# MrinalJain17/CT-image-segmentation

Hardware: AMD Instinct MI355X
Metric: CT volumes/sec training (512x512x48, bs=2/GPU) (higher is better)
Workload: dtype bf16; 1 GPU; 3D U-Net (MONAI UNet, channels 32-64-128-256, 2 res units) training step on 2x1x512x512x48 synthetic CT volumes per GPU (BASELINE.json configs[2]), CrossEntropy + Dice metric + Adam; global_batch=2, parallelism=dp1

## Files before the change

ct-image-segmentation_amd/csrc/conv_halo_sw.hip:

```cpp
#include "conv_common.h"

#ifndef SW_STORE8
#define SW_STORE8 0
#endif
#ifndef SW_FULL_WAIT
#define SW_FULL_WAIT 0
#endif
#ifndef SW_ABL
#define SW_ABL 0
#endif

namespace ctseg {

constexpr int SW_NTHR = 512, SW_TAPB = 8192;

template <int VB, bool UP> struct SwCfg {
  static constexpr bool DENSE = UP && VB == 256;
  static constexpr int TA = (VB == 128 || DENSE) ? 4 : 2;
  static constexpr int O = DENSE ? 1 : 0;
  static constexpr int LB = 10 - O;
  static constexpr int HV = DENSE ? 456 : (TA + 2) * 100;
  static constexpr int NPL = VB / 16, PLANE = HV * 16, HALO = NPL * PLANE;
  static constexpr int CG = VB / 2, CN = SW_TAPB / VB;
  static constexpr int NT = CN / 16;
  static constexpr int RT = TA / 2;
  static constexpr int KS = CG / 32;
  static constexpr int G = DENSE ? 2 : 3;
  static constexpr int NSTAGE = (27 + G - 1) / G;
  static constexpr int WRING = 2 * G * SW_TAPB;
  static constexpr int TOTAL = HALO + WRING + 8 * 3 * CN * 4 + 128 * 4 + 2 * CN * 4;
  static_assert(TOTAL <= 160 * 1024, "LDS");
  __host__ __device__ static constexpr int slot(int ha, int hb, int hc) { return ((ha - O) * LB + (hb - O)) * 10 + hc; }
};

struct SwGeom : TileAxes {};

template <typename H, int VB, bool UP, bool STATS, bool BST = false>
__global__ __launch_bounds__(SW_NTHR) void conv_halo_sw_kernel(const ConvKArgs P, const SwGeom G, int total_tiles) {
  static_assert(!BST || (!STATS && ((UP && VB == 256) || (!UP && VB == 128))), "backward statistics: the input-gradient passes this kernel takes");
  using CF = SwCfg<VB, UP>;
  constexpr int TA = CF::TA, NPL = CF::NPL, PLANE = CF::PLANE, CN = CF::CN, NT = CF::NT, RT = CF::RT, KS = CF::KS;
  constexpr int SW_G = CF::G, SW_NSTAGE = CF::NSTAGE;
  constexpr int O = UP ? 1 : 0;
  constexpr int FA = TA + 2 - O, FB = 10 - O, FV = FA * FB * FB;
  constexpr int NCH = FV * NPL, J = (NCH + SW_NTHR - 1) / SW_NTHR;

  __shared__ __attribute__((aligned(16))) char smem[CF::TOTAL];
  char* const sH = smem;
  char* const sW = smem + CF::HALO;
  float* const sStats = reinterpret_cast<float*>(sW + CF::WRING);
  int* const sTab = reinterpret_cast<int*>(sStats + 8 * 3 * CN);
  float* const sBt = reinterpret_cast<float*>(sTab + 128);

  const int tid = threadIdx.x, lane = tid & 63, wave = tid >> 6;
  const int r16 = lane & 15, q4 = lane >> 4;

  if (tid < 32) {
    int d = 0, wo = 0, kp = 0, cl = 0;
    if (tid < 27) {
      int c = 0, first = 0;
      while (tid >= first + P.cls[c].ntaps) { first += P.cls[c].ntaps; ++c; }
      const int ti = tid - first;
      const int tp = P.cls[c].taps[ti];
      int dv[3] = {tap_dx(tp), tap_dy(tp), tap_dz(tp)};
      d = ((dv[G.pa] * CF::LB + dv[G.pb]) * 10 + dv[G.pc]) * 16;
      wo = (int)(P.cls[c].w_off + (int64_t)ti * CF::CG);
      kp = P.cls[c].kpad;
      cl = c | ((ti == P.cls[c].ntaps - 1) ? 256 : 0);
    }
    sTab[tid] = d; sTab[32 + tid] = wo; sTab[64 + tid] = kp; sTab[96 + tid] = cl;
  }

  constexpr bool LEAN = BST;
  static_assert(!LEAN || (SW_NTHR / 8) % NPL == 0, "lean staging: the plane of a slot must not depend on j");
  int g_byte[LEAN ? 1 : J], g_habc[J], g_lds[LEAN ? 1 : J];
  const int pl0 = (tid >> 3) % NPL;
#pragma unroll
  for (int j = 0; j < J; ++j) {
    const int idx = tid + j * SW_NTHR;
    const int pl = (idx >> 3) % NPL, fv = (idx / (8 * NPL)) * 8 + (idx & 7);
    const int fa = fv / (FB * FB), rem = fv - fa * (FB * FB), fb = rem / FB, fc = rem - fb * FB;
    const int ha = fa + O, hb = fb + O, hc = fc + O;
    g_habc[j] = (fv < FV) ? (ha | (hb << 8) | (hc << 16)) : 0x7f7f7f;
    if constexpr (!LEAN) {
      g_byte[j] = (((ha - 1) * G.ia + (hb - 1) * G.ib + (hc - 1) * G.ic) * P.g_ld + pl * 8) * 2;
      g_lds[j] = pl * PLANE + CF::slot(ha, hb, hc) * 16;
    }
  }
  auto lean_habc = [&](int j, int& ha, int& hb, int& hc) {
    int h = g_habc[j];
    asm volatile("" : "+v"(h));
    ha = h & 0xff; hb = (h >> 8) & 0xff; hc = h >> 16;
  };
  const int64_t in_sample = (int64_t)P.Xi * P.Yi * P.Zi, out_sample = (int64_t)P.Xo * P.Yo * P.Zo;
  u32x4 rh[J];
  auto gload = [&](int t) {
    const auto [n, a0, b0, c0] = tile_origin_abc<TA>(t, G);
    const char* base = P.in + (n * in_sample + (int64_t)a0 * G.ia + (int64_t)b0 * G.ib + (int64_t)c0 * G.ic) * P.g_ld * 2;
#pragma unroll
    for (int j = 0; j < J; ++j) {
      const int ai = a0 - 1 + (g_habc[j] & 0xff), bi = b0 - 1 + ((g_habc[j] >> 8) & 0xff), ci = c0 - 1 + (g_habc[j] >> 16);
      u32x4 v = {0u, 0u, 0u, 0u};
      int gb;
      if constexpr (LEAN) {
        int ha, hb, hc;
        lean_habc(j, ha, hb, hc);
        gb = (((ha - 1) * G.ia + (hb - 1) * G.ib + (hc - 1) * G.ic) * P.g_ld + pl0 * 8) * 2;
      } else {
        gb = g_byte[j];
      }
      if (!(SW_ABL & 16) && (unsigned)ai < (unsigned)G.da && (unsigned)bi < (unsigned)G.db && (unsigned)ci < (unsigned)G.dc)
        v = *reinterpret_cast<const u32x4*>(base + gb);
      rh[j] = v;
    }
  };
  auto sstore = [&]() {
#pragma unroll
    for (int j = 0; j < J; ++j) {
      int gl;
      if constexpr (LEAN) {
        int ha, hb, hc;
        lean_habc(j, ha, hb, hc);
        gl = pl0 * PLANE + CF::slot(ha, hb, hc) * 16;
      } else {
        gl = g_lds[j];
      }
      if ((g_habc[j] & 0xff) != 0x7f) *reinterpret_cast<u32x4*>(sH + gl) = rh[j];
    }
  };

  typedef const __attribute__((address_space(1))) void* gptr_t;
  typedef __attribute__((address_space(3))) void* lptr_t;
  const int w_s64 = tid / (CN * 8), w_row = (tid >> 3) % CN, w_q8 = (tid & 7) ^ ((w_row >> 1) & 7);
  const int w_koff = w_s64 * 64 + w_q8 * 8;
  int wstage = 0;
  auto wload = [&](int stage_in_tile, int slot) {
    char* dst = sW + slot * (SW_G * SW_TAPB) + wave * 1024;
#pragma unroll
    for (int g = 0; g < SW_G; ++g) {
      const int tap = stage_in_tile * SW_G + g;
      if (SW_G * SW_NSTAGE > 27 && tap >= 27) continue;
      if (SW_ABL & 4) continue;
      const char* src = P.w + ((int64_t)sTab[32 + tap] + (int64_t)w_row * sTab[64 + tap] + w_koff) * 2;
      __builtin_amdgcn_global_load_lds((gptr_t)src, (lptr_t)(dst + g * SW_TAPB), 16, 0, 0);
    }
  };

  int pdb, pc;
  patch_voxel(r16, pdb, pc);
  int abase[RT], va[RT], vb[RT];
#pragma unroll
  for (int rt = 0; rt < RT; ++rt) {
    const int wa = (TA == 4) ? (wave >> 1) : (wave >> 2);
    const int i = (TA == 4) ? (2 * (wave & 1) + rt) : (wave & 3);
    va[rt] = wa;
    vb[rt] = 2 * i + pdb;
    abase[rt] = CF::slot(wa + 1, vb[rt] + 1, pc + 1) * 16 + q4 * PLANE;
  }
  const int wrd = r16 * 128, wswz = (r16 >> 1) & 7;
  const bool af32 = P.add_f32 != 0;
  const int ASZ = af32 ? 4 : 2;
  float bias[NT][4];
#pragma unroll
  for (int j = 0; j < NT; ++j)
#pragma unroll
    for (int e = 0; e < 4; ++e) bias[j][e] = (!BST && P.bias != nullptr) ? P.bias[j * 16 + 4 * q4 + e] : 0.f;

  float wsum[NT][4], wsq[NT][4];
#pragma unroll
  for (int j = 0; j < NT; ++j)
#pragma unroll
    for (int e = 0; e < 4; ++e) { wsum[j][e] = 0.f; wsq[j][e] = 0.f; }
  int stat_n = -1;
  auto flush_stats = [&](int n) {
#pragma unroll
    for (int j = 0; j < NT; ++j)
#pragma unroll
      for (int e = 0; e < 4; ++e) {
        float a = wsum[j][e], b = wsq[j][e];
        sum16(a, b);
        if (r16 == 0) {
          const int c = j * 16 + 4 * q4 + e;
          sStats[(wave * 2 + 0) * CN + c] = a;
          sStats[(wave * 2 + 1) * CN + c] = b;
        }
        wsum[j][e] = 0.f;
        wsq[j][e] = 0.f;
      }
    __syncthreads();
    if (tid < 2 * CN) {
      const int which = tid / CN, c = tid % CN;
      float a = 0.f;
#pragma unroll
      for (int w = 0; w < 8; ++w) a += sStats[(w * 2 + which) * CN + c];
      P.stats[stats_slot(P, n, blockIdx.x, which) + c] = a;
    }
    __syncthreads();
  };

  f32x4 acc[RT][NT];
  auto zero_acc = [&]() {
#pragma unroll
    for (int rt = 0; rt < RT; ++rt)
#pragma unroll
      for (int j = 0; j < NT; ++j) acc[rt][j] = f32x4{0.f, 0.f, 0.f, 0.f};
  };
  const int out_sample_bytes = (int)(out_sample * P.o_ld * 2), add_sample_bytes = (int)(out_sample * P.add_ld * ASZ);
  const bool apf = UP && !STATS && P.add != nullptr && !af32;
  int ooff[RT], aoff[RT];
#pragma unroll
  for (int rt = 0; rt < RT; ++rt) {
    const int vox = va[rt] * G.oa + vb[rt] * G.ob + pc * G.oc;
    ooff[rt] = (vox * P.o_ld + 4 * q4) * 2;
    aoff[rt] = (vox * P.add_ld + 4 * q4) * ASZ;
  }
  u32x2 apre[RT][NT];
  constexpr int NQ = NT / 2;
  f32x2 q1[NQ][4], q2[NQ][4];
  float q3 = 0.f;
#pragma unroll
  for (int jp = 0; jp < NQ; ++jp)
#pragma unroll
    for (int h = 0; h < 4; ++h) { q1[jp][h] = f32x2{0.f, 0.f}; q2[jp][h] = f32x2{0.f, 0.f}; }
  const float q_al = BST ? P.bst.alpha[0] : 1.f;
  const int ychunk = (q4 & 1) * 2 + (q4 >> 1);
  const int y_sample_bytes = BST ? (int)(out_sample * P.bst.y_ld * 2) : 0;
  int yoffc[RT];
#pragma unroll
  for (int rt = 0; rt < RT; ++rt) yoffc[rt] = BST ? ((va[rt] * G.oa + vb[rt] * G.ob + pc * G.oc) * P.bst.y_ld + ychunk * 8) * 2 : 0;
  u32x4 ypre[RT];
  int bst_n = -1;
  auto bst_consts = [&](int n) {
    if (tid < 2 * CN) {
      const int c = tid % CN, which = tid / CN;
      const float mean = P.bst.mr[((int64_t)n * P.bst.C + c) * 2], rstd = P.bst.mr[((int64_t)n * P.bst.C + c) * 2 + 1];
      sBt[which * CN + c] = which == 0 ? rstd : -mean * rstd;
    }
    __syncthreads();
  };
  auto bst_chunk = [&](int jp, const u32x4& gz, const u32x4& yv) {
    if (SW_ABL & 128) { q3 += __uint_as_float(gz[0] ^ yv[3]); return; }
    const float* const cb = sBt + jp * 32 + ychunk * 8;
    const f32x4 rs0 = *reinterpret_cast<const f32x4*>(cb), rs1 = *reinterpret_cast<const f32x4*>(cb + 4);
    const f32x4 nm0 = *reinterpret_cast<const f32x4*>(cb + CN), nm1 = *reinterpret_cast<const f32x4*>(cb + CN + 4);
    bst_pair_bf16(gz[0], yv[0], f32x2{rs0[0], rs0[1]}, f32x2{nm0[0], nm0[1]}, q_al, q1[jp][0], q2[jp][0], q3);
    bst_pair_bf16(gz[1], yv[1], f32x2{rs0[2], rs0[3]}, f32x2{nm0[2], nm0[3]}, q_al, q1[jp][1], q2[jp][1], q3);
    bst_pair_bf16(gz[2], yv[2], f32x2{rs1[0], rs1[1]}, f32x2{nm1[0], nm1[1]}, q_al, q1[jp][2], q2[jp][2], q3);
    bst_pair_bf16(gz[3], yv[3], f32x2{rs1[2], rs1[3]}, f32x2{nm1[2], nm1[3]}, q_al, q1[jp][3], q2[jp][3], q3);
  };
  auto flush_bst = [&](int n) {
#pragma unroll
    for (int jp = 0; jp < NQ; ++jp)
#pragma unroll
      for (int h = 0; h < 4; ++h)
#pragma unroll
        for (int e = 0; e < 2; ++e) {
          float a = q1[jp][h][e], b = q2[jp][h][e];
          sum16(a, b);
          if (r16 == 0) {
            sStats[(wave * 3 + 0) * CN + jp * 32 + ychunk * 8 + 2 * h + e] = a;
            sStats[(wave * 3 + 1) * CN + jp * 32 + ychunk * 8 + 2 * h + e] = b;
          }
          q1[jp][h][e] = 0.f; q2[jp][h][e] = 0.f;
        }
    {
      float c = q3;
      sum16(c);
      if (r16 == 0) sStats[(wave * 3 + 2) * CN + ychunk * 8] = c;
      q3 = 0.f;
    }
    __syncthreads();
    if (tid < 3 * CN) {
      const int which = tid / CN, c = tid % CN;
      float a = 0.f;
      if (which < 2 || ((c & 7) == 0 && c < 32)) {
#pragma unroll
        for (int w = 0; w < 8; ++w) a += sStats[(w * 3 + which) * CN + c];
      }
      P.bst.part[bst_slot(P.bst, n, blockIdx.x, which) + c] = a;
    }
    __syncthreads();
  };
  int pend = 0;
  auto class_base = [&](int cls, int a0, int b0, int c0) -> int {
    const ctseg_conv_class& K = P.cls[cls];
    return a0 * G.oa + b0 * G.ob + c0 * G.oc + (K.ox * P.Yo + K.oy) * P.Zo + K.oz;
  };
  auto add_issue = [&](int cls, int n, int a0, int b0, int c0) {
    const int cb = cls >= 0 ? class_base(cls, a0, b0, c0) : 0;
    if (apf) {
      const __amdgpu_buffer_rsrc_t ars = buffer_rsrc(P.add + (int64_t)n * add_sample_bytes, add_sample_bytes);
      const int soff = cb * P.add_ld * ASZ;
#pragma unroll
      for (int rt = 0; rt < RT; ++rt) {
        const bool rv = cls >= 0 && (a0 + va[rt] < G.da) && (b0 + vb[rt] < G.db) && (c0 + pc < G.dc);
#pragma unroll
        for (int j = 0; j < NT; ++j)
          apre[rt][j] = (SW_ABL & 32) ? u32x2{0u, 0u} : __builtin_amdgcn_raw_buffer_load_b64(ars, rv ? aoff[rt] + j * 16 * ASZ : (int)0x80000000, soff, 0);
      }
      pend += RT * NT;
    }
    if constexpr (BST) {
      const __amdgpu_buffer_rsrc_t yrs = buffer_rsrc(P.bst.y + (int64_t)n * y_sample_bytes, y_sample_bytes);
      const int soff = cb * P.bst.y_ld * 2;
#pragma unroll
      for (int rt = 0; rt < RT; ++rt) {
        const bool rv = cls >= 0 && (a0 + va[rt] < G.da) && (b0 + vb[rt] < G.db) && (c0 + pc < G.dc);
        ypre[rt] = (SW_ABL & 64) ? u32x4{1u, 2u, 3u, (uint32_t)soff} : __builtin_amdgcn_raw_buffer_load_b128(yrs, rv ? yoffc[rt] : (int)0x80000000, soff, 0);
      }
      pend += RT;
    }
  };
  auto epilogue = [&](int cls, int next_cls, int n, int a0, int b0, int c0) {
    const int cb = class_base(cls, a0, b0, c0);
    const __amdgpu_buffer_rsrc_t ors = buffer_rsrc(P.out + (int64_t)n * out_sample_bytes, out_sample_bytes);
    const int soff = cb * P.o_ld * 2;
    const int cbq = ((q4 & 1) * 2 + (q4 >> 1)) * 16;
#pragma unroll
    for (int rt = 0; rt < RT; ++rt) {
      const bool rv = (a0 + va[rt] < G.da) && (b0 + vb[rt] < G.db) && (c0 + pc < G.dc);
      u32x2 o2[NT];
#pragma unroll
      for (int j = 0; j < NT; ++j) {
        float v[4];
#pragma unroll
        for (int e = 0; e < 4; ++e) {
          v[e] = acc[rt][j][e] + bias[j][e];
          if (STATS && rv) { wsum[j][e] += v[e]; wsq[j][e] += v[e] * v[e]; }
        }
        if (apf) {
          const u32x2 w2 = apre[rt][j];
          v[0] += h2f<H>(w2[0] & 0xffffu); v[1] += h2f<H>(w2[0] >> 16); v[2] += h2f<H>(w2[1] & 0xffffu); v[3] += h2f<H>(w2[1] >> 16);
        } else if (P.add != nullptr && rv) {
          const char* ap = P.add + (int64_t)n * add_sample_bytes + (int64_t)cb * P.add_ld * ASZ + aoff[rt] + j * 16 * ASZ;
          if (af32) { const f32x4 a4 = *reinterpret_cast<const f32x4*>(ap); v[0] += a4[0]; v[1] += a4[1]; v[2] += a4[2]; v[3] += a4[3]; }
          else {
            const u32x2 w2 = *reinterpret_cast<const u32x2*>(ap);
            v[0] += h2f<H>(w2[0] & 0xffffu); v[1] += h2f<H>(w2[0] >> 16); v[2] += h2f<H>(w2[1] & 0xffffu); v[3] += h2f<H>(w2[1] >> 16);
          }
        }
        o2[j] = u32x2{pack2<H>(v[0], v[1]), pack2<H>(v[2], v[3])};
      }
#if SW_STORE8
#pragma unroll
      for (int j = 0; j < NT; ++j)
        __builtin_amdgcn_raw_buffer_store_b64(o2[j], ors, rv ? ooff[rt] + j * 32 : (int)0x80000000, soff, 0);
      continue;
#endif
#pragma unroll
      for (int jp = 0; jp < NT / 2; ++jp) {
        const auto s0 = __builtin_amdgcn_permlane16_swap(o2[2 * jp][0], o2[2 * jp + 1][0], false, false);
        const auto s1 = __builtin_amdgcn_permlane16_swap(o2[2 * jp][1], o2[2 * jp + 1][1], false, false);
        const u32x4 o4 = {s0[0], s1[0], s0[1], s1[1]};
        const bool keep = rv && (!(SW_ABL & 8) || o4[0] == 0x12345u);
        __builtin_amdgcn_raw_buffer_store_b128(o4, ors, keep ? ooff[rt] - 4 * q4 * 2 + jp * 64 + cbq : (int)0x80000000, soff, 0);
        asm volatile("s_nop 1" ::"v"(o4));
        if constexpr (BST) bst_chunk(jp, rv ? o4 : u32x4{0u, 0u, 0u, 0u}, ypre[rt]);
      }
    }
    pend += RT * NT / 2;
    if (apf || BST) add_issue(next_cls, n, a0, b0, c0);
  };
  auto stage_barrier = [&]() {
    constexpr int YL = BST ? RT : 0, E1 = RT * NT / 2 + YL, E2 = RT * NT / 2 + RT * NT + YL;
    constexpr int T1 = YL, T2 = RT * NT + YL;
    if (SW_FULL_WAIT || pend == 0) asm volatile("s_waitcnt vmcnt(0) lgkmcnt(0)" ::: "memory");
    else if (BST && pend == T1) asm volatile("s_waitcnt vmcnt(%0) lgkmcnt(0)" ::"n"(T1) : "memory");
    else if (BST && pend == T2) asm volatile("s_waitcnt vmcnt(%0) lgkmcnt(0)" ::"n"(T2) : "memory");
    else if (BST && pend == T1 + E1) asm volatile("s_waitcnt vmcnt(%0) lgkmcnt(0)" ::"n"(T1 + E1) : "memory");
    else if (BST && pend == T2 + E2) asm volatile("s_waitcnt vmcnt(%0) lgkmcnt(0)" ::"n"(T2 + E2) : "memory");
    else if (pend == E1) asm volatile("s_waitcnt vmcnt(%0) lgkmcnt(0)" ::"n"(E1) : "memory");
    else if (pend == 2 * E1) asm volatile("s_waitcnt vmcnt(%0) lgkmcnt(0)" ::"n"(2 * E1) : "memory");
    else if (pend == E2) asm volatile("s_waitcnt vmcnt(%0) lgkmcnt(0)" ::"n"(E2) : "memory");
    else if (pend == 2 * E2) asm volatile("s_waitcnt vmcnt(%0) lgkmcnt(0)" ::"n"(2 * E2) : "memory");
    else asm volatile("s_waitcnt vmcnt(0) lgkmcnt(0)" ::: "memory");
    __builtin_amdgcn_s_barrier();
    asm volatile("" ::: "memory");
    pend = 0;
  };

  auto epilogue_plain = [&](int cls, int n, int a0, int b0, int c0) {
    const ctseg_conv_class& K = P.cls[cls];
    int ov[3] = {K.ox, K.oy, K.oz};
    const int64_t obase = n * out_sample + (int64_t)a0 * G.oa + (int64_t)b0 * G.ob + (int64_t)c0 * G.oc +
                          ((int64_t)ov[0] * P.Yo + ov[1]) * P.Zo + ov[2];
#pragma unroll
    for (int rt = 0; rt < RT; ++rt) {
      const bool rv = (a0 + va[rt] < G.da) && (b0 + vb[rt] < G.db) && (c0 + pc < G.dc);
      const int64_t vox = obase + (int64_t)va[rt] * G.oa + (int64_t)vb[rt] * G.ob + (int64_t)pc * G.oc;
#pragma unroll
      for (int j = 0; j < NT; ++j) {
        const int ch = j * 16 + 4 * q4;
        float v[4];
#pragma unroll
        for (int e = 0; e < 4; ++e) {
          v[e] = acc[rt][j][e] + bias[j][e];
          if (STATS && rv) { wsum[j][e] += v[e]; wsq[j][e] += v[e] * v[e]; }
        }
        if (rv) {
          if (P.add != nullptr) {
            const char* ap = P.add + (vox * P.add_ld + ch) * ASZ;
            if (af32) { const f32x4 a4 = *reinterpret_cast<const f32x4*>(ap); v[0] += a4[0]; v[1] += a4[1]; v[2] += a4[2]; v[3] += a4[3]; }
            else {
              const u32x2 w2 = *reinterpret_cast<const u32x2*>(ap);
              v[0] += h2f<H>(w2[0] & 0xffffu); v[1] += h2f<H>(w2[0] >> 16); v[2] += h2f<H>(w2[1] & 0xffffu); v[3] += h2f<H>(w2[1] >> 16);
            }
          }
          *reinterpret_cast<u32x2*>(P.out + (vox * P.o_ld + ch) * 2) = u32x2{pack2<H>(v[0], v[1]), pack2<H>(v[2], v[3])};
        }
      }
    }
  };

  auto epilogue_plain_bst = [&](int n, int a0, int b0, int c0) {
    const ctseg_conv_class& K = P.cls[0];
    const int cb = a0 * G.oa + b0 * G.ob + c0 * G.oc + (K.ox * P.Yo + K.oy) * P.Zo + K.oz;
    const __amdgpu_buffer_rsrc_t ors = buffer_rsrc(P.out + (int64_t)n * out_sample_bytes, out_sample_bytes);
    const __amdgpu_buffer_rsrc_t yrs = buffer_rsrc(P.bst.y + (int64_t)n * y_sample_bytes, y_sample_bytes);
    u32x4 yq[RT][NQ];
#pragma unroll
    for (int rt = 0; rt < RT; ++rt) {
      const bool rv = (a0 + va[rt] < G.da) && (b0 + vb[rt] < G.db) && (c0 + pc < G.dc);
#pragma unroll
      for (int jp = 0; jp < NQ; ++jp) yq[rt][jp] = __builtin_amdgcn_raw_buffer_load_b128(yrs, rv ? yoffc[rt] + jp * 64 : (int)0x80000000, cb * P.bst.y_ld * 2, 0);
    }
    const int cbq = ychunk * 16;
#pragma unroll
    for (int rt = 0; rt < RT; ++rt) {
      const bool rv = (a0 + va[rt] < G.da) && (b0 + vb[rt] < G.db) && (c0 + pc < G.dc);
      u32x2 o2[NT];
#pragma unroll
      for (int j = 0; j < NT; ++j) {
        float v[4];
#pragma unroll
        for (int e = 0; e < 4; ++e) v[e] = acc[rt][j][e];
        if (P.add != nullptr && rv) {
          const char* ap = P.add + (int64_t)n * add_sample_bytes + (int64_t)cb * P.add_ld * ASZ + aoff[rt] + j * 16 * ASZ;
          if (af32) { const f32x4 a4 = *reinterpret_cast<const f32x4*>(ap); v[0] += a4[0]; v[1] += a4[1]; v[2] += a4[2]; v[3] += a4[3]; }
          else {
            const u32x2 w2 = *reinterpret_cast<const u32x2*>(ap);
            v[0] += h2f<H>(w2[0] & 0xffffu); v[1] += h2f<H>(w2[0] >> 16); v[2] += h2f<H>(w2[1] & 0xffffu); v[3] += h2f<H>(w2[1] >> 16);
          }
        }
        o2[j] = u32x2{pack2<H>(v[0], v[1]), pack2<H>(v[2], v[3])};
      }
#pragma unroll
      for (int jp = 0; jp < NQ; ++jp) {
        const auto s0 = __builtin_amdgcn_permlane16_swap(o2[2 * jp][0], o2[2 * jp + 1][0], false, false);
        const auto s1 = __builtin_amdgcn_permlane16_swap(o2[2 * jp][1], o2[2 * jp + 1][1], false, false);
        const u32x4 o4 = {s0[0], s1[0], s0[1], s1[1]};
        __builtin_amdgcn_raw_buffer_store_b128(o4, ors, rv ? ooff[rt] - 4 * q4 * 2 + jp * 64 + cbq : (int)0x80000000, cb * P.o_ld * 2, 0);
        asm volatile("s_nop 1" ::"v"(o4));
        bst_chunk(jp, rv ? o4 : u32x4{0u, 0u, 0u, 0u}, yq[rt][jp]);
      }
    }
  };

  const auto [first, stride, last] = xcd_tile_seq([] { return blockIdx.x; }, gridDim.x, total_tiles);

  __syncthreads();
  int t = first;
  if (t < last) {
    gload(t);
    wload(0, 0);
    sstore();
  }
  __syncthreads();
  for (; t < last; t += stride) {
    const int tn = t + stride;
    const auto [n, a0, b0, c0] = tile_origin_abc<TA>(t, G);
    if (STATS && n != stat_n) {
      if (stat_n >= 0) flush_stats(stat_n);
      stat_n = n;
    }
    if constexpr (BST) {
      if (n != bst_n) {
        if (bst_n >= 0) flush_bst(bst_n);
        bst_n = n;
        bst_consts(n);
      }
    }
    zero_acc();
#pragma unroll 1
    for (int s = 0; s < SW_NSTAGE; ++s) {
      const int slot = wstage & 1;
      if (s + 1 < SW_NSTAGE) wload(s + 1, slot ^ 1);
      else if (tn < last) wload(0, slot ^ 1);
      if (s == 0 && tn < last) gload(tn);
      if ((apf || BST) && s == 0) add_issue(sTab[96] & 255, n, a0, b0, c0);
      const char* wb = sW + slot * (SW_G * SW_TAPB) + wrd;
#pragma unroll
      for (int g = 0; g < SW_G; ++g) {
        const int tap = s * SW_G + g;
        if (SW_G * SW_NSTAGE > 27 && tap >= 27) continue;
        const int delta = sTab[tap];
#pragma unroll
        for (int ks = 0; ks < KS; ++ks) {
          u32x4 xf[RT], wf[NT];
#pragma unroll
          for (int rt = 0; rt < RT; ++rt)
            xf[rt] = (SW_ABL & 2) ? u32x4{(uint32_t)(delta + rt), 1u, 2u, (uint32_t)ks} : *reinterpret_cast<const u32x4*>(sH + abase[rt] + ks * 4 * PLANE + delta);
          const char* wk = wb + g * SW_TAPB + (ks >> 1) * (CN * 128) + (((4 * (ks & 1) + q4) ^ wswz) << 4);
#pragma unroll
          for (int j = 0; j < NT; ++j) wf[j] = (SW_ABL & 2) ? u32x4{(uint32_t)(j + g), 3u, (uint32_t)tap, 5u} : *reinterpret_cast<const u32x4*>(wk + j * 16 * 128);
#pragma unroll
          for (int rt = 0; rt < RT; ++rt)
#pragma unroll
            for (int j = 0; j < NT; ++j) {
              if constexpr ((SW_ABL & 1) != 0) acc[rt][j][0] += __builtin_bit_cast(f32x4, wf[j])[0] * __builtin_bit_cast(f32x4, xf[rt])[1];
              else mma16<H>(acc[rt][j], wf[j], xf[rt]);
            }
        }
        if constexpr (UP) {
          const int cl = sTab[96 + tap];
          if (cl & 256) {
            epilogue(cl & 255, tap + 1 < 27 ? (sTab[96 + tap + 1] & 255) : -1, n, a0, b0, c0);
            zero_acc();
          }
        }
      }
      ++wstage;
      if constexpr (UP) stage_barrier();
      else __syncthreads();
    }
    if constexpr (!UP && BST) epilogue_plain_bst(n, a0, b0, c0);
    else if constexpr (!UP) epilogue_plain(0, n, a0, b0, c0);
    if (tn < last) {
      sstore();
      __syncthreads();
    }
  }
  if (STATS && stat_n >= 0) flush_stats(stat_n);
  if constexpr (BST) { if (bst_n >= 0) flush_bst(bst_n); }
}

static void sw_geom(const ConvKArgs& a, int vb, SwGeom& g) {
  tile_axes_fill(g, a, (vb == 128 || a.sout == 2) ? 4 : 2, 2);
}

bool conv_halo_sw_eligible(const ConvKArgs& a, int dtype, int nclass) {
  if (!is16(dtype) || a.out_f32 || a.sin != 1) return false;
  const int vb = a.Cg * 2;
  if (!((vb == 128 && a.Cn == 64) || (vb == 256 && a.Cn == 32)) || a.Cn_store != a.Cn) return false;
  if ((a.g_ld % 8) != 0 || ((uintptr_t)a.in % 16) != 0 || ((uintptr_t)a.w % 16) != 0) return false;
  if (a.Xr != a.Xi || a.Yr != a.Yi || a.Zr != a.Zi) return false;
  if (sample_bytes(a.Xi, a.Yi, a.Zi, a.g_ld, 2) >= (1ll << 31)) return false;
  if ((int64_t)a.Xr * a.Yr * a.Zr < 2048) return false;
  const bool up = nclass == 8;
  if (up) {
    if (a.sout != 2 || a.Xo != 2 * a.Xr || a.Yo != 2 * a.Yr || a.Zo != 2 * a.Zr) return false;
  } else {
    if (nclass != 1 || a.sout != 1 || a.Xo != a.Xr || a.Yo != a.Yr || a.Zo != a.Zr) return false;
  }
  int taps = 0;
  for (int c = 0; c < nclass; ++c) {
    const ctseg_conv_class& k = a.cls[c];
    if (up ? (k.ntaps != (1 << __builtin_popcount(c))) : (k.ntaps != 27)) return false;
    if (k.kpad < k.ntaps * a.Cg || (k.kpad % 8) != 0 || (k.w_off % 8) != 0) return false;
    if (k.w_off + (int64_t)a.Cn * k.kpad >= (1ll << 31)) return false;
    taps += k.ntaps;
    if (!taps_within(k.taps, k.ntaps, up ? 0 : -1, 1)) return false;
  }
  return taps == 27;
}

static int sw_grid(const ConvKArgs& a, const SwGeom& g) {
  return persistent_grid(CTSEG_NUM_CU, g.tiles * a.N);
}

int conv_halo_sw_slots(const ConvKArgs& a) {
  SwGeom g;
  sw_geom(a, a.Cg * 2, g);
  return sw_grid(a, g);
}

int conv_halo_sw_bst_slots(const ConvKArgs& a, int nclass) {
  if (a.dtype != CTSEG_BF16 || a.stats != nullptr || a.bias != nullptr) return 0;
  if (!((nclass == 8 && a.Cg == 128) || (nclass == 1 && a.Cg == 64))) return 0;
  if (a.bst.C != a.Cn || a.bst.col0 != 0 || a.Cn_store != a.Cn || (a.o_ld % 8) != 0 || ((uintptr_t)a.out % 16) != 0) return 0;
  if ((a.bst.y_ld % 8) != 0 || ((uintptr_t)a.bst.y % 16) != 0) return 0;
  if (sample_bytes(a.Xo, a.Yo, a.Zo, a.bst.y_ld, 2) >= (1ll << 31) || sample_bytes(a.Xo, a.Yo, a.Zo, a.o_ld, 2) >= (1ll << 31)) return 0;
  return conv_halo_sw_slots(a);
}

void launch_conv_halo_sw(ConvKArgs& a, int nclass, hipStream_t st) {
  SwGeom g;
  const int vb = a.Cg * 2;
  sw_geom(a, vb, g);
  a.tiles = g.tiles;
  const int total = g.tiles * a.N;
  const dim3 grid((unsigned)sw_grid(a, g)), blk(SW_NTHR);
  const bool up = nclass == 8, stats = a.stats != nullptr;
  if (a.bst.part != nullptr) {
    if (up) hipLaunchKernelGGL((conv_halo_sw_kernel<BF16, 256, true, false, true>), grid, blk, 0, st, a, g, total);
    else hipLaunchKernelGGL((conv_halo_sw_kernel<BF16, 128, false, false, true>), grid, blk, 0, st, a, g, total);
    return;
  }
  with_storage(a.dtype, [&](auto h, auto vb128, auto up_, auto stats_) {
    constexpr int VB = decltype(vb128)::value ? 128 : 256;
    hipLaunchKernelGGL((conv_halo_sw_kernel<decltype(h), VB, decltype(up_)::value, decltype(stats_)::value>), grid, blk, 0, st, a, g, total);
  }, vb == 128, up, stats);
}

}
```

Measured before the change: 231.7 volumes/s.

## Use triple-buffered weight ring with counted vmcnt waits for plain VB128 conv

```diff
diff --git a/ct-image-segmentation_amd/csrc/conv_halo_sw.hip b/ct-image-segmentation_amd/csrc/conv_halo_sw.hip
--- a/ct-image-segmentation_amd/csrc/conv_halo_sw.hip
+++ b/ct-image-segmentation_amd/csrc/conv_halo_sw.hip
@@ -27,7 +27,8 @@
   static constexpr int KS = CG / 32;
   static constexpr int G = DENSE ? 2 : 3;
   static constexpr int NSTAGE = (27 + G - 1) / G;
-  static constexpr int WRING = 2 * G * SW_TAPB;
+  static constexpr int NSLOT = (!UP && VB == 128) ? 3 : 2;
+  static constexpr int WRING = NSLOT * G * SW_TAPB;
   static constexpr int TOTAL = HALO + WRING + 8 * 3 * CN * 4 + 128 * 4 + 2 * CN * 4;
   static_assert(TOTAL <= 160 * 1024, "LDS");
   __host__ __device__ static constexpr int slot(int ha, int hb, int hc) { return ((ha - O) * LB + (hb - O)) * 10 + hc; }
@@ -40,7 +41,8 @@
   static_assert(!BST || (!STATS && ((UP && VB == 256) || (!UP && VB == 128))), "backward statistics: the input-gradient passes this kernel takes");
   using CF = SwCfg<VB, UP>;
   constexpr int TA = CF::TA, NPL = CF::NPL, PLANE = CF::PLANE, CN = CF::CN, NT = CF::NT, RT = CF::RT, KS = CF::KS;
-  constexpr int SW_G = CF::G, SW_NSTAGE = CF::NSTAGE;
+  constexpr int SW_G = CF::G, SW_NSTAGE = CF::NSTAGE, NSLOT = CF::NSLOT;
+  constexpr bool RING3 = NSLOT == 3;
   constexpr int O = UP ? 1 : 0;
   constexpr int FA = TA + 2 - O, FB = 10 - O, FV = FA * FB * FB;
   constexpr int NCH = FV * NPL, J = (NCH + SW_NTHR - 1) / SW_NTHR;
@@ -94,8 +96,28 @@
   };
   const int64_t in_sample = (int64_t)P.Xi * P.Yi * P.Zi, out_sample = (int64_t)P.Xo * P.Yo * P.Zo;
   u32x4 rh[J];
-  auto gload = [&](int t) {
+  const int in_sample_bytes = (int)(in_sample * P.g_ld * 2);
+  auto gload = [&](int t, bool live = true) {
     const auto [n, a0, b0, c0] = tile_origin_abc<TA>(t, G);
+    if constexpr (RING3) {
+      const __amdgpu_buffer_rsrc_t irs = buffer_rsrc(P.in + n * in_sample * P.g_ld * 2, in_sample_bytes);
+      const int tb = (a0 * G.ia + b0 * G.ib + c0 * G.ic) * P.g_ld * 2;
+#pragma unroll
+      for (int j = 0; j < J; ++j) {
+        const int ai = a0 - 1 + (g_habc[j] & 0xff), bi = b0 - 1 + ((g_habc[j] >> 8) & 0xff), ci = c0 - 1 + (g_habc[j] >> 16);
+        int gb;
+        if constexpr (LEAN) {
+          int ha, hb, hc;
+          lean_habc(j, ha, hb, hc);
+          gb = (((ha - 1) * G.ia + (hb - 1) * G.ib + (hc - 1) * G.ic) * P.g_ld + pl0 * 8) * 2;
+        } else {
+          gb = g_byte[j];
+        }
+        const bool in = live && (unsigned)ai < (unsigned)G.da && (unsigned)bi < (unsigned)G.db && (unsigned)ci < (unsigned)G.dc;
+        rh[j] = (SW_ABL & 16) ? u32x4{0u, 0u, 0u, 0u} : __builtin_amdgcn_raw_buffer_load_b128(irs, in ? tb + gb : (int)0x80000000, 0, 0);
+      }
+      return;
+    }
     const char* base = P.in + (n * in_sample + (int64_t)a0 * G.ia + (int64_t)b0 * G.ib + (int64_t)c0 * G.ic) * P.g_ld * 2;
 #pragma unroll
     for (int j = 0; j < J; ++j) {
@@ -379,35 +401,57 @@
     pend = 0;
   };
 
+  constexpr int EP_ST = (!UP && BST) ? RT * NQ : RT * NT;
+  constexpr int EP_Y = (!UP && BST) ? RT * NQ : 0;
+  constexpr int EP_AD = (SW_ABL & 32) ? 0 : RT * NT;
   auto epilogue_plain = [&](int cls, int n, int a0, int b0, int c0) {
-    const ctseg_conv_class& K = P.cls[cls];
-    int ov[3] = {K.ox, K.oy, K.oz};
-    const int64_t obase = n * out_sample + (int64_t)a0 * G.oa + (int64_t)b0 * G.ob + (int64_t)c0 * G.oc +
-                          ((int64_t)ov[0] * P.Yo + ov[1]) * P.Zo + ov[2];
+    const int cb = class_base(cls, a0, b0, c0);
+    const __amdgpu_buffer_rsrc_t ors = buffer_rsrc(P.out + (int64_t)n * out_sample_bytes, out_sample_bytes);
+    const __amdgpu_buffer_rsrc_t ars = buffer_rsrc(P.add + (int64_t)n * add_sample_bytes, P.add != nullptr ? add_sample_bytes : 0);
+    const int so = cb * P.o_ld * 2, sa = cb * P.add_ld * ASZ;
+    const bool has_add = !(SW_ABL & 32) && P.add != nullptr;
+    u32x4 aq[RT][NT];
+    if (has_add && af32) {
+#pragma unroll
+      for (int rt = 0; rt < RT; ++rt) {
+        const bool rv = (a0 + va[rt] < G.da) && (b0 + vb[rt] < G.db) && (c0 + pc < G.dc);
+#pragma unroll
+        for (int j = 0; j < NT; ++j) aq[rt][j] = __builtin_amdgcn_raw_buffer_load_b128(ars, rv ? aoff[rt] + j * 16 * ASZ : (int)0x80000000, sa, 0);
+      }
+    } else if (has_add) {
+#pragma unroll
+      for (int rt = 0; rt < RT; ++rt) {
+        const bool rv = (a0 + va[rt] < G.da) && (b0 + vb[rt] < G.db) && (c0 + pc < G.dc);
+#pragma unroll
+        for (int j = 0; j < NT; ++j) {
+          const u32x2 w2 = __builtin_amdgcn_raw_buffer_load_b64(ars, rv ? aoff[rt] + j * 16 * ASZ : (int)0x80000000, sa, 0);
+          aq[rt][j] = u32x4{w2[0], w2[1], 0u, 0u};
+        }
+      }
+    }
 #pragma unroll
     for (int rt = 0; rt < RT; ++rt) {
       const bool rv = (a0 + va[rt] < G.da) && (b0 + vb[rt] < G.db) && (c0 + pc < G.dc);
-      const int64_t vox = obase + (int64_t)va[rt] * G.oa + (int64_t)vb[rt] * G.ob + (int64_t)pc * G.oc;
 #pragma unroll
       for (int j = 0; j < NT; ++j) {
-        const int ch = j * 16 + 4 * q4;
         float v[4];
 #pragma unroll
         for (int e = 0; e < 4; ++e) {
           v[e] = acc[rt][j][e] + bias[j][e];
-          if (STATS && rv) { wsum[j][e] += v[e]; wsq[j][e] += v[e] * v[e]; }
-        }
-        if (rv) {
-          if (P.add != nullptr) {
-            const char* ap = P.add + (vox * P.add_ld + ch) * ASZ;
-            if (af32) { const f32x4 a4 = *reinterpret_cast<const f32x4*>(ap); v[0] += a4[0]; v[1] += a4[1]; v[2] += a4[2]; v[3] += a4[3]; }
-            else {
-              const u32x2 w2 = *reinterpret_cast<const u32x2*>(ap);
-              v[0] += h2f<H>(w2[0] & 0xffffu); v[1] += h2f<H>(w2[0] >> 16); v[2] += h2f<H>(w2[1] & 0xffffu); v[3] += h2f<H>(w2[1] >> 16);
-            }
+          if (STATS && rv) { wsum[j][e] += v[e]; wsq[j][e] = fmaf(v[e], v[e], wsq[j][e]); }
+        }
+        if (has_add) {
+          const u32x4 w4 = aq[rt][j];
+          if (af32) {
+            const f32x4 a4 = __builtin_bit_cast(f32x4, w4);
+            v[0] += a4[0]; v[1] += a4[1]; v[2] += a4[2]; v[3] += a4[3];
+          } else {
+            v[0] += h2f<H>(w4[0] & 0xffffu); v[1] += h2f<H>(w4[0] >> 16); v[2] += h2f<H>(w4[1] & 0xffffu); v[3] += h2f<H>(w4[1] >> 16);
           }
-          *reinterpret_cast<u32x2*>(P.out + (vox * P.o_ld + ch) * 2) = u32x2{pack2<H>(v[0], v[1]), pack2<H>(v[2], v[3])};
-        }
+        }
+        const u32x2 o2 = {pack2<H>(v[0], v[1]), pack2<H>(v[2], v[3])};
+        const bool keep = rv && (!(SW_ABL & 8) || o2[0] == 0x12345u);
+        __builtin_amdgcn_raw_buffer_store_b64(o2, ors, keep ? ooff[rt] + j * 32 : (int)0x80000000, so, 0);
       }
     }
   };
@@ -417,12 +461,24 @@
     const int cb = a0 * G.oa + b0 * G.ob + c0 * G.oc + (K.ox * P.Yo + K.oy) * P.Zo + K.oz;
     const __amdgpu_buffer_rsrc_t ors = buffer_rsrc(P.out + (int64_t)n * out_sample_bytes, out_sample_bytes);
     const __amdgpu_buffer_rsrc_t yrs = buffer_rsrc(P.bst.y + (int64_t)n * y_sample_bytes, y_sample_bytes);
+    const __amdgpu_buffer_rsrc_t ars = buffer_rsrc(P.add + (int64_t)n * add_sample_bytes, P.add != nullptr ? add_sample_bytes : 0);
     u32x4 yq[RT][NQ];
 #pragma unroll
     for (int rt = 0; rt < RT; ++rt) {
       const bool rv = (a0 + va[rt] < G.da) && (b0 + vb[rt] < G.db) && (c0 + pc < G.dc);
 #pragma unroll
       for (int jp = 0; jp < NQ; ++jp) yq[rt][jp] = __builtin_amdgcn_raw_buffer_load_b128(yrs, rv ? yoffc[rt] + jp * 64 : (int)0x80000000, cb * P.bst.y_ld * 2, 0);
+    }
+    const bool has_add = !(SW_ABL & 32) && P.add != nullptr;
+    const int sa = cb * P.add_ld * ASZ;
+    u32x2 aq[RT][NT];
+    if (has_add && !af32) {
+#pragma unroll
+      for (int rt = 0; rt < RT; ++rt) {
+        const bool rv = (a0 + va[rt] < G.da) && (b0 + vb[rt] < G.db) && (c0 + pc < G.dc);
+#pragma unroll
+        for (int j = 0; j < NT; ++j) aq[rt][j] = __builtin_amdgcn_raw_buffer_load_b64(ars, rv ? aoff[rt] + j * 16 * ASZ : (int)0x80000000, sa, 0);
+      }
     }
     const int cbq = ychunk * 16;
 #pragma unroll
@@ -434,11 +490,12 @@
         float v[4];
 #pragma unroll
         for (int e = 0; e < 4; ++e) v[e] = acc[rt][j][e];
-        if (P.add != nullptr && rv) {
-          const char* ap = P.add + (int64_t)n * add_sample_bytes + (int64_t)cb * P.add_ld * ASZ + aoff[rt] + j * 16 * ASZ;
-          if (af32) { const f32x4 a4 = *reinterpret_cast<const f32x4*>(ap); v[0] += a4[0]; v[1] += a4[1]; v[2] += a4[2]; v[3] += a4[3]; }
-          else {
-            const u32x2 w2 = *reinterpret_cast<const u32x2*>(ap);
+        if (has_add) {
+          if (af32) {
+            const f32x4 a4 = __builtin_bit_cast(f32x4, __builtin_amdgcn_raw_buffer_load_b128(ars, rv ? aoff[rt] + j * 16 * ASZ : (int)0x80000000, sa, 0));
+            v[0] += a4[0]; v[1] += a4[1]; v[2] += a4[2]; v[3] += a4[3];
+          } else {
+            const u32x2 w2 = aq[rt][j];
             v[0] += h2f<H>(w2[0] & 0xffffu); v[1] += h2f<H>(w2[0] >> 16); v[2] += h2f<H>(w2[1] & 0xffffu); v[3] += h2f<H>(w2[1] >> 16);
           }
         }
@@ -458,14 +515,38 @@
 
   const auto [first, stride, last] = xcd_tile_seq([] { return blockIdx.x; }, gridDim.x, total_tiles);
 
+  constexpr int WD = (SW_ABL & 4) ? 0 : SW_G, HJN = (SW_ABL & 16) ? 0 : J, EP0 = EP_ST + EP_Y, EP1 = EP0 + EP_AD;
+  auto ring_wait = [&](int n) {
+#define SW_VMW(k) asm volatile("s_waitcnt vmcnt(%0) lgkmcnt(0)" ::"n"(k) : "memory")
+    static_assert(EP1 + WD + HJN < 64, "vmcnt is a 6-bit counter");
+    if (SW_FULL_WAIT || n <= 0) SW_VMW(0);
+    else if (n == WD) SW_VMW(WD);
+    else if (n == WD + HJN) SW_VMW(WD + HJN);
+    else if (n == EP0 + WD + HJN) SW_VMW(EP0 + WD + HJN);
+    else if (n == EP1 + WD + HJN) SW_VMW(EP1 + WD + HJN);
+    else SW_VMW(0);
+#undef SW_VMW
+    __builtin_amdgcn_s_barrier();
+    asm volatile("" ::: "memory");
+  };
+  const int ep_ops = P.add != nullptr ? EP1 : EP0;
+  int ep_prev = 0;
+
   __syncthreads();
   int t = first;
   if (t < last) {
     gload(t);
+    if constexpr (RING3) asm volatile("" ::: "memory");
     wload(0, 0);
+    if constexpr (RING3) {
+      asm volatile("" ::: "memory");
+      wload(1, 1);
+      asm volatile("" ::: "memory");
+    }
     sstore();
   }
-  __syncthreads();
+  if constexpr (RING3) ring_wait(t < last ? WD : 0);
+  else __syncthreads();
   for (; t < last; t += stride) {
     const int tn = t + stride;
     const auto [n, a0, b0, c0] = tile_origin_abc<TA>(t, G);
@@ -481,13 +562,27 @@
       }
     }
     zero_acc();
+    if constexpr (RING3) {
+      wload(2, wstage == 0 ? 2 : wstage - 1);
+      asm volatile("" ::: "memory");
+      gload(tn < last ? tn : t, tn < last);
+      asm volatile("" ::: "memory");
+    }
 #pragma unroll 1
     for (int s = 0; s < SW_NSTAGE; ++s) {
-      const int slot = wstage & 1;
-      if (s + 1 < SW_NSTAGE) wload(s + 1, slot ^ 1);
-      else if (tn < last) wload(0, slot ^ 1);
-      if (s == 0 && tn < last) gload(tn);
-      if ((apf || BST) && s == 0) add_issue(sTab[96] & 255, n, a0, b0, c0);
+      const int slot = RING3 ? wstage : (wstage & 1);
+      if constexpr (RING3) {
+        const int ahead = slot == 0 ? 2 : slot - 1;
+        if (s == 0) {}
+        else if (s + 2 < SW_NSTAGE) wload(s + 2, ahead);
+        else if (tn < last) wload(s + 2 - SW_NSTAGE, ahead);
+        asm volatile("" ::: "memory");
+      } else {
+        if (s + 1 < SW_NSTAGE) wload(s + 1, slot ^ 1);
+        else if (tn < last) wload(0, slot ^ 1);
+        if (s == 0 && tn < last) gload(tn);
+      }
+      if (UP && (apf || BST) && s == 0) add_issue(sTab[96] & 255, n, a0, b0, c0);
       const char* wb = sW + slot * (SW_G * SW_TAPB) + wrd;
 #pragma unroll
       for (int g = 0; g < SW_G; ++g) {
@@ -520,8 +615,24 @@
         }
       }
       ++wstage;
-      if constexpr (UP) stage_barrier();
+      if constexpr (RING3) {
+        if (wstage == NSLOT) wstage = 0;
+        ring_wait(s == 0 ? ep_prev + WD + HJN : (s < SW_NSTAGE - 2 || tn < last) ? WD : 0);
+      } else if constexpr (UP) stage_barrier();
       else __syncthreads();
+    }
+    if constexpr (RING3) {
+      sstore();
+      asm volatile("" ::: "memory");
+      if constexpr (BST) epilogue_plain_bst(n, a0, b0, c0);
+      else epilogue_plain(0, n, a0, b0, c0);
+      ep_prev = ep_ops;
+      if (tn < last) {
+        asm volatile("s_waitcnt lgkmcnt(0)" ::: "memory");
+        __builtin_amdgcn_s_barrier();
+        asm volatile("" ::: "memory");
+      }
+      continue;
     }
     if constexpr (!UP && BST) epilogue_plain_bst(n, a0, b0, c0);
     else if constexpr (!UP) epilogue_plain(0, n, a0, b0, c0);
@@ -551,6 +662,8 @@
     if (a.sout != 2 || a.Xo != 2 * a.Xr || a.Yo != 2 * a.Yr || a.Zo != 2 * a.Zr) return false;
   } else {
     if (nclass != 1 || a.sout != 1 || a.Xo != a.Xr || a.Yo != a.Yr || a.Zo != a.Zr) return false;
+    if (sample_bytes(a.Xo, a.Yo, a.Zo, a.o_ld, 2) >= (1ll << 31)) return false;
+    if (a.add != nullptr && sample_bytes(a.Xo, a.Yo, a.Zo, a.add_ld, a.add_f32 ? 4 : 2) >= (1ll << 31)) return false;
   }
   int taps = 0;
   for (int c = 0; c < nclass; ++c) {
```

Result: no change. 231.6 volumes/s, median of 2 (-0.1%).
